# hip-satomi/microbeSEG

Measured on AMD Instinct MI355X. Metric: training crops/sec (256px), higher is better.
Workload: dtype f32; 1 GPU; BASELINE configs[1]: DU-Net distance-map training step, filters [64, 1024], 256x256 crops, per-GPU batch 32, fp32, relu/bn, SmoothL1x2 + Adam(amsgrad); global_batch=32, parallelism=dp1, launch=eager

## Files before the change

include/mseg_hip.h:

```cpp
#ifndef MSEG_HIP_H
#define MSEG_HIP_H

#include <stddef.h>
#include <stdint.h>

#ifdef __cplusplus
extern "C" {
#endif

#define MSEG_OK 0
#define MSEG_EINVAL (-1)
#define MSEG_ELAUNCH (-2)
#define MSEG_EWORKSPACE (-3)

#define MSEG_ACT_NONE 0
#define MSEG_ACT_RELU 1
#define MSEG_ACT_LEAKY 2
#define MSEG_ACT_ELU 3
#define MSEG_ACT_MISH 4

#define MSEG_NORM_BN 0
#define MSEG_NORM_GN 1
#define MSEG_NORM_IN 2

// ... 120 lines not shown
                        const float* running_var, float eps, int C, float* scale, float* shift, void* stream);
int mseg_norm_bwd(const void* gy, const void* z, int N, int HW, int C, int st, int act, int norm, const float* gamma,
                  const float* mean, const float* rstd, void* dz, float* dgamma, float* dbeta, float* dbias,
                  const void* act_in , void* ws, void* stream);

int mseg_maxpool2x2_fwd(const MsegSrc* src, int N, int H, int W, float* out, void* stream);
int mseg_maxpool2x2_bwd(const MsegSrc* src, int N, int H, int W, const float* gout, float* gin, int accumulate,
                        void* stream);

int mseg_head_fwd(const MsegSrc* src, int N, int HW, const float* w, const float* b, int Co, float* out_nchw,
                  void* stream);
size_t mseg_head_bwd_workspace_bytes(int N, int HW, int C, int Co);
int mseg_head_bwd(const MsegSrc* src, int N, int HW, const float* w, int Co, const float* gout_nchw, void* gy,
                  int gy_dtype , float* dW, float* db, void* ws,
                  void* stream);

int mseg_softmax3_hwc(const float* logits_chw, int Hp, int Wp, int pad_y, int pad_x, float* probs_hwc, void* stream);

size_t mseg_loss_workspace_bytes(size_t n);
int mseg_regression_loss(const float* pred, const float* target, size_t n, int kind, float* loss_out,
                         void* ws, void* stream);
int mseg_regression_loss_bwd(const float* pred, const float* target, size_t n, int kind, const float* gscale_dev,
                             float* grad, void* stream);
int mseg_ce_dice_fwd(const float* logits, const int64_t* labels, int N, int HW, int with_dice, double* sums6,
                     double* ce_sum, void* ws, void* stream);
int mseg_ce_dice_bwd(const float* logits, const int64_t* labels, int N, int HW, int with_dice, const double* sums6,
                     double total_px, double dice_weight, const float* gscale_dev, float* grad, void* stream);

int mseg_polygons_find(const uint16_t* labels, int H, int W, int32_t* cand_px, int32_t* cand_id, int32_t* cand_len,
                       int capacity, int32_t* n_cand_dev, void* stream);
// ... 136 lines not shown
```

microbeseg_amd/_lib.py:

```python
import ctypes as C
import os
import pathlib

_HERE = pathlib.Path(__file__).resolve().parent
LIB_PATH = _HERE / "libmseg_hip.so"

ACT = {"none": 0, "relu": 1, "leakyrelu": 2, "elu": 3, "mish": 4}
NORM = {"bn": 0, "gn": 1, "in": 2}
MODE_CONV, MODE_TCONV = 0, 1
EPI_PLAIN, EPI_SCATTER2X2 = 0, 1
MORDER_LINEAR, MORDER_PARITY = 0, 1
ST_F32, ST_BF16 = 0, 1
PIX_U8, PIX_U16, PIX_I32, PIX_F32 = 0, 1, 2, 3
GATHER_RAW, GATHER_F32, GATHER_NORM, GATHER_I64 = 0, 1, 2, 3


class MsegLibraryError(RuntimeError):
    pass


class MsegSrc(C.Structure):
    _fields_ = [("ptr", C.c_void_p), ("scale", C.c_void_p), ("shift", C.c_void_p),
                ("C", C.c_int32), ("act", C.c_int32), ("ss", C.c_int32), ("dtype", C.c_int32)]

# ... 67 lines not shown
    "mseg_pack_job_blocks": (C.c_uint, [_I, _I, _I]),
    "mseg_pack_weights_multi": (_I, [_P, _I, C.c_uint, _P]),
    "mseg_norm_workspace_bytes": (_SZ, [_I, _I, _I]),
    "mseg_norm_set_tails": (_I, [_I]),
    "mseg_norm_set_finish": (_I, [_I]),
    "mseg_norm_stats_from_conv": (_I, [_P, _I, _I, C.c_longlong, _P, _P, _F, _P, _P, _P, _P, _P, _P, _F, _P, _P]),
    "mseg_norm_stats": (_I, [_P, _I, _I, _I, _I, _I, _I, _P, _P, _F, _P, _P, _P, _P, _P, _P, _F, _P, _P, _P]),
    "mseg_activation": (_I, [_P, _I, _I, _I, _I, _I, _P, _P]),
    "mseg_bn_eval_coeffs": (_I, [_P, _P, _P, _P, _F, _I, _P, _P, _P]),
    "mseg_norm_bwd": (_I, [_P, _P, _I, _I, _I, _I, _I, _I, _P, _P, _P, _P, _P, _P, _P, _P, _P, _P]),
    "mseg_maxpool2x2_fwd": (_I, [C.POINTER(MsegSrc), _I, _I, _I, _P, _P]),
    "mseg_maxpool2x2_bwd": (_I, [C.POINTER(MsegSrc), _I, _I, _I, _P, _P, _I, _P]),
    "mseg_head_fwd": (_I, [C.POINTER(MsegSrc), _I, _I, _P, _P, _I, _P, _P]),
    "mseg_head_bwd_workspace_bytes": (_SZ, [_I, _I, _I, _I]),
    "mseg_head_bwd": (_I, [C.POINTER(MsegSrc), _I, _I, _P, _I, _P, _P, _I, _P, _P, _P, _P]),
    "mseg_softmax3_hwc": (_I, [_P, _I, _I, _I, _I, _P, _P]),
    "mseg_loss_workspace_bytes": (_SZ, [_SZ]),
    "mseg_regression_loss": (_I, [_P, _P, _SZ, _I, _P, _P, _P]),
    "mseg_regression_loss_bwd": (_I, [_P, _P, _SZ, _I, _P, _P, _P]),
    "mseg_ce_dice_fwd": (_I, [_P, _P, _I, _I, _I, _P, _P, _P, _P]),
    "mseg_ce_dice_bwd": (_I, [_P, _P, _I, _I, _I, _P, C.c_double, C.c_double, _P, _P, _P]),
    "mseg_adam_amsgrad_step": (_I, [_P, _P, _P, _P, _P, _SZ, _D, _D, _D, _D, _I, _P]),
    "mseg_adam_amsgrad_step_dev": (_I, [_P, _P, _P, _P, _P, _SZ, _P, _D, _D, _D, _P]),
    "mseg_ranger_step": (_I, [_P, _P, _P, _P, _P, _SZ, _I, _D, _D, _D, _D, _I, _I, _I, _D, _P]),
    "mseg_ranger_step_multi": (_I, [_P, _I, _D, _D, _D, _D, _P]),
    "mseg_postproc_workspace_bytes": (_SZ, [_I, _I]),
    "mseg_postproc_tuning": (_I, [_I, _I, _I]),
    "mseg_postproc_set_const_stream": (_I, [_I]),
    "mseg_distance_postprocess": (_I, [_P, _P, _I, _I, _F, _F, _I, _P, _P, _P, _P, _SZ, _P]),
    "mseg_boundary_postprocess": (_I, [_P, _I, _I, _P, _P, _P, _P, _SZ, _P]),
# ... 92 lines not shown
```

microbeseg_amd/csrc/common.h:

```cpp
#pragma once
#include <hip/hip_runtime.h>
#include <stdint.h>
#include "../../include/mseg_hip.h"

extern "C" void mseg_set_hip_error(int e);
extern "C" int mseg_dispatch_dry(void);

#define MSEG_LAUNCH_CHECK()                           \
  do {                                                \
    if (mseg_dispatch_dry()) break;                   \
    hipError_t e__ = hipGetLastError();               \
    if (e__ != hipSuccess) {                          \
      mseg_set_hip_error((int)e__);                   \
      return MSEG_ELAUNCH;                            \
    }                                                 \
  } while (0)

extern "C" void mseg_note_launch(const char* kernel, unsigned grid, unsigned block, int aux);
extern "C" void mseg_dispatch_begin(int dry);
extern "C" void mseg_dispatch_end(MsegKernelInfo* info);
extern "C" void mseg_dispatch_note(int precision, size_t workspace);
extern "C" void mseg_dispatch_note_stats(int rows);
#define MSEG_KL(K, grid_, block_, shmem_, st_, ...)                                              \
  do {                                                                                           \
// ... 152 lines not shown
__device__ __forceinline__ float raw_frame_norm(unsigned v, float fmin, float frange) {
  return __fsub_rn(__fdiv_rn(__fmul_rn(2.f, __fsub_rn((float)v, fmin)), frange), 1.f);
}

__device__ __forceinline__ unsigned xcd_logical_id(unsigned hw_id, unsigned nwg) {
  const unsigned q = nwg >> 3, r = nwg & 7u, xcd = hw_id & 7u;
  return (xcd < r ? xcd * (q + 1u) : r * (q + 1u) + (xcd - r) * q) + (hw_id >> 3);
}

__device__ __forceinline__ float clamp_lo(float v, float lo) {
  float r;
  asm("v_max_f32 %0, %1, %2" : "=v"(r) : "v"(v), "v"(lo));
  return r;
}

__device__ __forceinline__ double wave_sum(double v) {
#pragma unroll
  for (int o = 32; o > 0; o >>= 1) v += __shfl_xor(v, o, 64);
  return v;
}
```

microbeseg_amd/csrc/head.hip:

```cpp
#include "common.h"

#define HEAD_MAXCO 4

template <bool S16, int CO>
__global__ __launch_bounds__(256) void head_fwd_kernel(const MsegSrc s, int N, int HW, const float* __restrict__ w,
                                                       const float* __restrict__ b, int Co, int lpp,
                                                       float* __restrict__ out) {
  constexpr int V = S16 ? 8 : 4, U = 4;
  const int CV = s.C / V;
  const long long total = (long long)N * HW;
  const int sub = threadIdx.x % lpp;
  const long long ppb = blockDim.x / lpp;
  for (long long base = (long long)blockIdx.x * ppb * U; base < total; base += (long long)gridDim.x * ppb * U) {
    float acc[U][CO];
#pragma unroll
    for (int u = 0; u < U; ++u)
#pragma unroll
      for (int co = 0; co < CO; ++co) acc[u][co] = 0.f;
    for (int cv = sub; cv < CV; cv += lpp) {
      uint4 raw[U];
#pragma unroll
      for (int u = 0; u < U; ++u) {
        const long long pix = base + u * ppb + threadIdx.x / lpp;
        const size_t e = (size_t)(pix < total ? pix : 0) * s.C + cv * V;
// ... 157 lines not shown
          float yv[V], o[V];
          if (S16) {
            yv[0] = bf16_lo(yraw[u].x); yv[1] = bf16_hi(yraw[u].x); yv[2] = bf16_lo(yraw[u].y); yv[3] = bf16_hi(yraw[u].y);
            yv[V - 4] = bf16_lo(yraw[u].z); yv[V - 3] = bf16_hi(yraw[u].z); yv[V - 2] = bf16_lo(yraw[u].w); yv[V - 1] = bf16_hi(yraw[u].w);
          } else {
            yv[0] = __uint_as_float(yraw[u].x); yv[1] = __uint_as_float(yraw[u].y);
            yv[2] = __uint_as_float(yraw[u].z); yv[3] = __uint_as_float(yraw[u].w);
          }
#pragma unroll
          for (int j = 0; j < V; j += 4) {
            const float4 a = act_fwd4(make_float4(yv[j], yv[j + 1], yv[j + 2], yv[j + 3]), s.act);
            yv[j] = a.x; yv[j + 1] = a.y; yv[j + 2] = a.z; yv[j + 3] = a.w;
          }
          if (s.scale) {
#pragma unroll
            for (int j = 0; j < V; ++j) yv[j] = yv[j] * sc[j] + sh[j];
          }
#pragma unroll
          for (int j = 0; j < V; ++j) o[j] = 0.f;
#pragma unroll
          for (int co = 0; co < CO; ++co) {
            if (co < g.Co) {
              const float gvc = gv[u][co];
#pragma unroll
              for (int j = 0; j < V; ++j) {
                o[j] += gvc * wv[co][j];
                dw[co][j] += (double)gvc * yv[j];
              }
              if (cv == 0) dbs[co] += gvc;
            }
          }
          if (V == 8 && gy_dtype == MSEG_ST_BF16) {
            *reinterpret_cast<uint4*>(reinterpret_cast<uint16_t*>(gy) + off) =
                make_uint4(pack_bf16x2(o[0], o[1]), pack_bf16x2(o[2], o[3]), pack_bf16x2(o[V - 4], o[V - 3]),
                           pack_bf16x2(o[V - 2], o[V - 1]));
          } else {
#pragma unroll
            for (int j = 0; j < V; j += 4) st_f4_rt(gy, off + j, make_float4(o[j], o[j + 1], o[j + 2], o[j + 3]), gy_dtype);
          }
        }
      }
    }
#pragma unroll
// ... 44 lines not shown
  const int i = blockIdx.x * 8 + o;
  double s = 0.0;
  if (i < total) {
    const int slot = (i < g.Co * g.C) ? i : HEAD_MAXCO * g.C + (i - g.Co * g.C);
    for (int k = kg; k < blocks; k += 32) s += part[(size_t)k * per + slot];
  }
  red[kg][o] = s;
  __syncthreads();
  if (kg == 0 && i < total) {
    double t = 0.0;
#pragma unroll
    for (int j = 0; j < 32; ++j) t += red[j][o];
    if (i < g.Co * g.C) dW[i] = (float)t;
    else if (db) db[i - g.Co * g.C] = (float)t;
  }
}

extern "C" int mseg_head_bwd(const MsegSrc* src, int N, int HW, const float* w, int Co, const float* gout_nchw,
                             void* gy, int gy_dtype, float* dW, float* db, void* ws, void* stream) {
  if (!src || !src->ptr || !w || !gout_nchw || !gy || !dW || !ws) return MSEG_EINVAL;
  if (gy_dtype != MSEG_ST_F32 && gy_dtype != MSEG_ST_BF16) return MSEG_EINVAL;
  if (N <= 0 || HW <= 0 || Co <= 0 || Co > HEAD_MAXCO || src->C <= 0 || (src->C & 3)) return MSEG_EINVAL;
  HeadGeom g = head_geom(N, HW, src->C, Co);
  hipStream_t st = (hipStream_t)stream;
#define HEAD_BWD(CO_, U_, S16_) hipLaunchKernelGGL((head_bwd_kernel<CO_, U_, S16_>), dim3(g.chunks, N), dim3(256), 0, st, *src, g, \
                                                   w, gout_nchw, gy, gy_dtype, (double*)ws)
  if (src->dtype == MSEG_ST_BF16) {
    if (src->C & 7) return MSEG_EINVAL;
    if (Co == 1) HEAD_BWD(1, 2, true); else if (Co == 2) HEAD_BWD(2, 2, true); else HEAD_BWD(4, 1, true);
  } else {
    if (Co == 1) HEAD_BWD(1, 4, false); else if (Co == 2) HEAD_BWD(2, 2, false); else HEAD_BWD(4, 1, false);
  }
#undef HEAD_BWD
  MSEG_LAUNCH_CHECK();
  hipLaunchKernelGGL(head_bwd_reduce_kernel, dim3((Co * (src->C + 1) + 7) / 8), dim3(256), 0, st,
                     (const double*)ws, g, dW, db);
  MSEG_LAUNCH_CHECK();
  return MSEG_OK;
}

__global__ void softmax3_hwc_kernel(const float* __restrict__ logits, int Hp, int Wp, int py, int px, int H, int W,
                                    float* __restrict__ probs) {
  const size_t n = (size_t)H * W;
  const size_t i = (size_t)blockIdx.x * blockDim.x + threadIdx.x;
  if (i >= n) return;
  const int y = (int)(i / W), x = (int)(i - (size_t)y * W);
  const size_t src = (size_t)(y + py) * Wp + (x + px);
  const size_t plane = (size_t)Hp * Wp;
  const float l0 = logits[src], l1 = logits[plane + src], l2 = logits[2 * plane + src];
  const float m = fmaxf(l0, fmaxf(l1, l2));
  const float e0 = expf(l0 - m), e1 = expf(l1 - m), e2 = expf(l2 - m);
// ... 16 lines not shown
```

microbeseg_amd/csrc/norm.hip:

```cpp
#include "common.h"
#include <stdlib.h>

struct NormGeom {
  int N, HW, C, chunks, rows_per_chunk;
  int cw, slices;
};

#define NORM_CTR_BYTES 65536
#define NORM_CTR_MAX (NORM_CTR_BYTES / 4)

static NormGeom norm_geom(int N, int HW, int C, int vec = 4) {
  NormGeom g;
  g.N = N; g.HW = HW; g.C = C;
  const int C4 = C / vec;
  g.cw = C4 < 16 ? (C4 > 0 ? C4 : 1) : 16;
  g.slices = (C4 + g.cw - 1) / g.cw;
  const int rpi = 256 / g.cw;
  const int min_rows = 8 * rpi;
  const int target = 1024;
  int want = (target + N * g.slices - 1) / (N * g.slices > 0 ? N * g.slices : 1);
  int chunks = HW / min_rows;
  if (chunks > want) chunks = want;
  if (chunks < 1) chunks = 1;
  g.rows_per_chunk = (HW + chunks - 1) / chunks;
// ... 365 lines not shown
        }
      } else {
        const double mu = t.mean[c2], r = t.rstd[c2], ga = t.gamma ? (double)t.gamma[c2] : 1.0;
        const double sx = r * (b0 - mu * a0);
        const double m1 = ga * a0 / cnt, m2 = ga * sx / cnt;
        t.k1[c2] = (float)(ga * r);
        t.k2[c2] = (float)(-r * r * m2);
        t.k3[c2] = (float)(-r * m1 + r * r * m2 * mu);
        if (t.dgamma) t.dgamma[c2] = (float)sx;
        if (t.dbeta) t.dbeta[c2] = (float)a0;
      }
    }
  }
}

__device__ __forceinline__ void norm_reduce_chunks_body(const double* __restrict__ part, double* __restrict__ nc,
                                                        const NormGeom& g, int ns, bool handoff, double (*red)[32]) {
  const int o = threadIdx.x & 31, kg = threadIdx.x >> 5;
  const int total = ns * g.N * g.C;
  for (int base = blockIdx.x * 32; base < total; base += gridDim.x * 32) {
    const int i = base + o;
    double acc = 0.0;
    int c = 0, n = 0, sidx = 0;
    if (i < total) {
      c = i % g.C;
      n = (i / g.C) % g.N;
      sidx = i / (g.C * g.N);
      for (int k = kg; k < g.chunks; k += 8) acc += part[(((size_t)n * g.chunks + k) * 3 + sidx) * g.C + c];
    }
    red[kg][o] = acc;
// ... 419 lines not shown
            (const float*)nullptr, 0, g, act, (double*)nullptr, aio_, t);
  MSEG_LAUNCH_CHECK();
  return MSEG_OK;
}

extern "C" int mseg_bn_eval_coeffs(const float* gamma, const float* beta, const float* running_mean,
                                   const float* running_var, float eps, int C, float* scale, float* shift,
                                   void* stream) {
  if (!running_mean || !running_var || !scale || !shift || C <= 0) return MSEG_EINVAL;
  hipLaunchKernelGGL(bn_eval_coeffs_kernel, dim3((C + 255) / 256), dim3(256), 0, (hipStream_t)stream, gamma, beta,
                     running_mean, running_var, eps, C, scale, shift);
  MSEG_LAUNCH_CHECK();
  return MSEG_OK;
}

extern "C" int mseg_norm_bwd(const void* gy, const void* z, int N, int HW, int C, int st_, int act, int norm,
                             const float* gamma, const float* mean, const float* rstd, void* dz, float* dgamma,
                             float* dbeta, float* dbias, const void* act_in, void* ws, void* stream) {
  if (!gy || !z || !mean || !rstd || !dz || !ws || N <= 0 || HW <= 0 || C <= 0 || (C & 3)) return MSEG_EINVAL;
  if ((st_ != MSEG_ST_F32 && st_ != MSEG_ST_BF16) || (st_ == MSEG_ST_BF16 && (C & 7))) return MSEG_EINVAL;
  if (norm < 0 || norm > 2) return MSEG_EINVAL;
  if (norm == MSEG_NORM_GN && (C % 8)) return MSEG_EINVAL;
  hipStream_t st = (hipStream_t)stream;
  NormGeom g = norm_geom(N, HW, C, norm_vec(st_));
  double* part = (double*)((char*)ws + NORM_CTR_BYTES);
  double* nc = part + (size_t)N * g.chunks * 3 * C;
  float* k1 = (float*)(nc + (size_t)3 * N * C);
  float* k2 = k1 + (size_t)N * C;
  float* k3 = k2 + (size_t)N * C;
  const int kss = (norm == MSEG_NORM_BN) ? 0 : C;
  const bool tails = norm_tails_fit(g);
  NormTail t = {};
  t.kind = (tails && norm == MSEG_NORM_BN) ? NORM_TAIL_BN_BWD : NORM_TAIL_NONE;
  t.norm = norm; t.ctr = (unsigned*)ws; t.nc = nc; t.gamma = gamma; t.mean = mean; t.rstd = rstd;
  t.k1 = k1; t.k2 = k2; t.k3 = k3; t.dgamma = dgamma; t.dbeta = dbeta;
  NORM_PASS(1, const_cast<void*>(act_in), z, gy, (void*)nullptr, (const float*)nullptr, (const float*)nullptr,
            (const float*)nullptr, 0, g, act, part, aio_, t);
  MSEG_LAUNCH_CHECK();
  if (t.kind == NORM_TAIL_NONE && norm == MSEG_NORM_BN && norm_finish_fits(C)) {
    NormTail tf = t;
    tf.kind = NORM_TAIL_BN_BWD;
    norm_launch_finish((const double*)part, nc, g, 2, tf, N, C, st);
    MSEG_LAUNCH_CHECK();
  } else if (t.kind == NORM_TAIL_NONE) {
    hipLaunchKernelGGL(norm_reduce_chunks_kernel, dim3(nblocks((size_t)2 * N * C * 8, 4096u)), dim3(256), 0, st,
                       (const double*)part, nc, g, 2);
    MSEG_LAUNCH_CHECK();
    hipLaunchKernelGGL(norm_bwd_finalize_kernel, dim3(nblocks(norm == MSEG_NORM_BN ? C : (size_t)N * C)), dim3(256), 0,
                       st, (const double*)nc, g, norm, gamma, mean, rstd, k1, k2, k3, dgamma, dbeta);
    MSEG_LAUNCH_CHECK();
  }
  double* part2 = part;
  NormTail t2 = {};
  t2.kind = (tails && dbias) ? NORM_TAIL_COLSUM : NORM_TAIL_NONE;
  t2.norm = norm; t2.ctr = (unsigned*)ws; t2.nc = nc; t2.colsum = dbias;
  NORM_PASS(2, const_cast<void*>(act_in), z, gy, dz, (const float*)k1, (const float*)k2, (const float*)k3, kss, g, act,
            part2, aio_, t2);
  MSEG_LAUNCH_CHECK();
  if (dbias && t2.kind == NORM_TAIL_NONE && norm_finish_fits(C)) {
    NormTail tf = t2;
    tf.kind = NORM_TAIL_COLSUM;
    norm_launch_finish((const double*)part2, nc, g, 1, tf, N, C, st);
    MSEG_LAUNCH_CHECK();
  } else if (dbias && t2.kind == NORM_TAIL_NONE) {
    hipLaunchKernelGGL(norm_reduce_chunks_kernel, dim3(nblocks((size_t)N * C * 8, 4096u)), dim3(256), 0, st,
                       (const double*)part2, nc, g, 1);
    MSEG_LAUNCH_CHECK();
    hipLaunchKernelGGL(norm_colsum_kernel, dim3(nblocks(C)), dim3(256), 0, st, (const double*)nc, g, dbias);
    MSEG_LAUNCH_CHECK();
  }
  return MSEG_OK;
}

__global__ void maxpool_fwd_kernel(const MsegSrc s, int N, int H, int W, float* __restrict__ out) {
  const int Ho = H >> 1, Wo = W >> 1, C4 = s.C >> 2;
  const size_t total = (size_t)N * Ho * Wo * C4;
  for (size_t i = (size_t)blockIdx.x * blockDim.x + threadIdx.x; i < total; i += (size_t)gridDim.x * blockDim.x) {
    const int c = (int)(i % C4) * 4;
    size_t r = i / C4;
    const int x = (int)(r % Wo); r /= Wo;
    const int y = (int)(r % Ho);
    const int n = (int)(r / Ho);
    float4 best;
#pragma unroll
    for (int k = 0; k < 4; ++k) {
      const size_t pix = ((size_t)n * H + 2 * y + (k >> 1)) * W + 2 * x + (k & 1);
      float4 v = *reinterpret_cast<const float4*>(s.ptr + pix * s.C + c);
      v = src_transform4(v, s, n, c);
// ... 68 lines not shown
```

microbeseg_amd/engine.py:

```python
import ctypes as C
import os

import torch

from . import _lib
from ._lib import (ACT, NORM, MODE_CONV, MODE_TCONV, EPI_PLAIN, EPI_SCATTER2X2, MORDER_LINEAR, MORDER_PARITY,
                   ST_F32, ST_BF16, MsegSrc, MsegIgemm, MsegWgrad, MsegKernelInfo, check)

BN_EPS = 1e-5
BN_MOMENTUM = 0.1


def _ptr(t):
    return None if t is None else t.data_ptr()


def _stream():
    return torch.cuda.current_stream().cuda_stream


def _pad4(c):
    return (c + 3) // 4 * 4


def _st(t):
    return ST_BF16 if t.dtype == torch.bfloat16 else ST_F32


class Node:
    __slots__ = ("z", "a", "N", "H", "W", "C", "act", "norm", "scale", "shift", "ss", "mean", "rstd", "layer", "inputs",
                 "grad")

    def __init__(self, z, N, H, W, C):
        self.z, self.N, self.H, self.W, self.C = z, N, H, W, C
        self.a = None
        self.act, self.norm = 0, None
        self.scale = self.shift = self.mean = self.rstd = None
        self.ss = 0
        self.layer, self.inputs, self.grad = None, (), None

    def src(self, transform=True):
        s = MsegSrc()
        s.ptr = self.z.data_ptr()
        s.C = self.C
        s.dtype = _st(self.z)
        if transform:
            if self.a is not None:
                s.ptr = self.a.data_ptr()
                s.act = ACT["none"]
            else:
                s.act = self.act
            s.scale = _ptr(self.scale)
            s.shift = _ptr(self.shift)
            s.ss = self.ss
# ... 531 lines not shown
                                  node.rstd.data_ptr(), _ptr(running_mean), _ptr(running_var), BN_MOMENTUM,
                                  _ptr(node.a), w.data_ptr(), _stream()), "norm_stats")
    if running_mean is not None:
        torch.autograd.graph.increment_version((running_mean, running_var))
        note_training_step()


def norm_bwd(node, gy, gamma, dgamma, dbeta, dbias, ws):
    lib = _lib.load()
    N, HW, Cc = node.N, node.H * node.W, node.C
    w = ws.get("norm", lib.mseg_norm_workspace_bytes(N, HW, Cc), zero=True)
    check(lib.mseg_norm_bwd(gy.data_ptr(), node.z.data_ptr(), N, HW, Cc, _st(node.z), node.act, node.norm, _ptr(gamma),
                            node.mean.data_ptr(), node.rstd.data_ptr(), gy.data_ptr(), _ptr(dgamma), _ptr(dbeta),
                            _ptr(dbias), _ptr(node.a), w.data_ptr(), _stream()), "norm_bwd")
    return gy


class ConvSpec:

    def __init__(self, kind, conv, norm_mod, act, norm):
        self.kind = kind
        self.conv = conv
        self.norm_mod = norm_mod
        self.act = ACT[act]
        self.norm = NORM[norm]

    def params(self):
        ps = [self.conv.weight, self.conv.bias]
        if self.norm in (NORM["bn"], NORM["gn"]):
            ps += [self.norm_mod.weight, self.norm_mod.bias]
# ... 269 lines not shown


_wgrad_overlap = os.environ.get("MSEG_WGRAD_OVERLAP", "1") != "0"
_side_streams = {}


def set_wgrad_overlap(flag):
    global _wgrad_overlap
    _wgrad_overlap = bool(flag)


def get_wgrad_overlap():
    return _wgrad_overlap


_overlap_in_capture = os.environ.get("MSEG_OVERLAP_IN_CAPTURE", "0") == "1"


_decoder_overlap = os.environ.get("MSEG_DECODER_OVERLAP", "0") == "1"


def set_decoder_overlap(flag):
    global _decoder_overlap
    _decoder_overlap = bool(flag)


def get_decoder_overlap():
    return _decoder_overlap


# ... 32 lines not shown
    def on_side(dz, fn):
        if side is None:
            return fn(ws)
        ev = torch.cuda.Event()
        ev.record(main)
        with torch.cuda.stream(side):
            side.wait_event(ev)
            fn(_SideWs(ws))
        held.append(dz)
        held_bytes[0] += dz.numel() * dz.element_size()
        if held_bytes[0] > _SIDE_HOLD_BYTES:
            main.wait_stream(side)
            held.clear()
            held_bytes[0] = 0

    for (head, node), go in zip(tape.heads, grad_outs):
        hc = head.conv
        co = hc.weight.shape[0]
        if go is None:
            go = torch.zeros((node.N, co, node.H, node.W), dtype=torch.float32, device=node.z.device)
        go = go.contiguous().float()
        gy = torch.empty_like(node.z)
        dW = _grad_buf(hc.weight, direct)
        db = _grad_buf(hc.bias, direct)
        w = ws.get("head", lib.mseg_head_bwd_workspace_bytes(node.N, node.H * node.W, node.C, co))
        s = node.src()
        check(lib.mseg_head_bwd(C.byref(s), node.N, node.H * node.W, hc.weight.detach().data_ptr(), co,
                                go.data_ptr(), gy.data_ptr(), _st(gy), dW.data_ptr(), db.data_ptr(), w.data_ptr(),
                                _stream()), "head_bwd")
        assert node.grad is None
        node.grad = gy
        grads[id(hc.weight)] = dW
        grads[id(hc.bias)] = db
        if on_grads is not None:
            on_grads([dW, db])

    for node in reversed(tape.nodes):
        sp = node.layer
        gy = node.grad
        node.grad = None
        if gy is None:
            raise RuntimeError("internal: node without gradient")
        if sp is _MaxPoolMarker:
            i0 = node.inputs[0]
            tgt, acc = _accumulate_target(i0, None)
            s = i0.src()
            check(lib.mseg_maxpool2x2_bwd(C.byref(s), i0.N, i0.H, i0.W, gy.data_ptr(), tgt.data_ptr(), acc, _stream()),
                  "maxpool_bwd")
            continue
        conv = sp.conv
        nm = sp.norm_mod
        has_affine = sp.norm in (NORM["bn"], NORM["gn"])
        dgamma = _grad_buf(nm.weight, direct) if has_affine else None
        dbeta = _grad_buf(nm.bias, direct) if has_affine else None
        dbias = _grad_buf(conv.bias, direct)
        dz = norm_bwd(node, gy, nm.weight.detach() if has_affine else None, dgamma, dbeta, dbias, ws)
        if has_affine:
            grads[id(nm.weight)] = dgamma
            grads[id(nm.bias)] = dbeta
        grads[id(conv.bias)] = dbias
        wt = conv.weight.detach()
        dW = _grad_buf(conv.weight, direct)
        ins = node.inputs
        i0 = ins[0]
        N = node.N
        if sp.kind == "up":
            cin, cout = wt.shape[0], wt.shape[1]
            on_side(dz, lambda w_, i0=i0, dz=dz, dW=dW, cout=cout, node=node: wgrad(
                i0.src(), [plain_src(dz, cout)], dW, N, i0.H, i0.W, node.H, node.W, 2, 2, 2, 0, w_))
            wp = pack_weight(conv.weight, 4, cin, cout, 1, cout * 4, 4, kind="dgrad")
            tgt, acc = _accumulate_target(i0, None)
# ... 92 lines not shown
```

Baseline: 244.3 crops/s.

## Fuse head 1x1-conv backward into final norm backward passes

Adds a fused head+norm backward path. The head's input gradient (gout·W) is recomputed on the fly inside the norm statistics and apply kernels instead of being materialized as a full gy tensor. The head weight and bias gradients are accumulated in the same stats pass. This removes one full-resolution write and read of gy and one separate head-backward kernel at the largest 256x256 resolution. The cost is extra per-element FMA work that is done twice, a larger workspace that must be zero-initialized, and eligibility checks in the backward schedule.

New measurement: 245.3 crops/s (median of 6 runs). About the same (+0.4%).

```diff
diff --git a/include/mseg_hip.h b/include/mseg_hip.h
--- a/include/mseg_hip.h
+++ b/include/mseg_hip.h
@@ -158,6 +158,12 @@
 int mseg_head_bwd(const MsegSrc* src, int N, int HW, const float* w, int Co, const float* gout_nchw, void* gy,
                   int gy_dtype , float* dW, float* db, void* ws,
                   void* stream);
+
+size_t mseg_head_norm_bwd_workspace_bytes(int N, int HW, int C, int Co);
+int mseg_head_norm_bwd(const float* gout_nchw, const float* w, int Co, const float* scale, const float* shift, int ss,
+                       const void* z, int N, int HW, int C, int st, int act, int norm, const float* gamma, const float* mean,
+                       const float* rstd, void* dz, float* dgamma, float* dbeta, float* dbias, float* dW_head, float* db_head,
+                       const void* act_in, void* ws, void* stream);
 
 int mseg_softmax3_hwc(const float* logits_chw, int Hp, int Wp, int pad_y, int pad_x, float* probs_hwc, void* stream);
 
diff --git a/microbeseg_amd/_lib.py b/microbeseg_amd/_lib.py
--- a/microbeseg_amd/_lib.py
+++ b/microbeseg_amd/_lib.py
@@ -105,6 +105,9 @@
     "mseg_head_fwd": (_I, [C.POINTER(MsegSrc), _I, _I, _P, _P, _I, _P, _P]),
     "mseg_head_bwd_workspace_bytes": (_SZ, [_I, _I, _I, _I]),
     "mseg_head_bwd": (_I, [C.POINTER(MsegSrc), _I, _I, _P, _I, _P, _P, _I, _P, _P, _P, _P]),
+    "mseg_head_norm_bwd_workspace_bytes": (_SZ, [_I, _I, _I, _I]),
+    "mseg_head_norm_bwd": (_I, [_P, _P, _I, _P, _P, _I, _P, _I, _I, _I, _I, _I, _I, _P, _P, _P, _P, _P, _P, _P, _P, _P, _P, _P,
+                                _P]),
     "mseg_softmax3_hwc": (_I, [_P, _I, _I, _I, _I, _P, _P]),
     "mseg_loss_workspace_bytes": (_SZ, [_SZ]),
     "mseg_regression_loss": (_I, [_P, _P, _SZ, _I, _P, _P, _P]),
diff --git a/microbeseg_amd/csrc/common.h b/microbeseg_amd/csrc/common.h
--- a/microbeseg_amd/csrc/common.h
+++ b/microbeseg_amd/csrc/common.h
@@ -190,6 +190,23 @@
   return r;
 }
 
+#define HEAD_MAXCO 4
+template <int CO, int V>
+__device__ __forceinline__ void head_gy(const float (&gv)[CO], const float (&wv)[CO][V], int Co, float (&o)[V]) {
+#pragma unroll
+  for (int j = 0; j < V; ++j) o[j] = 0.f;
+#pragma unroll
+  for (int co = 0; co < CO; ++co) {
+    if (co < Co) {
+      const float gvc = gv[co];
+#pragma unroll
+      for (int j = 0; j < V; ++j) o[j] = fmaf(gvc, wv[co][j], o[j]);
+    }
+  }
+}
+__attribute__((visibility("hidden"))) void head_bwd_reduce_launch(const double* part, int N, int chunks, int C, int Co,
+                                                                  float* dW, float* db, hipStream_t st);
+
 __device__ __forceinline__ double wave_sum(double v) {
 #pragma unroll
   for (int o = 32; o > 0; o >>= 1) v += __shfl_xor(v, o, 64);
diff --git a/microbeseg_amd/csrc/head.hip b/microbeseg_amd/csrc/head.hip
--- a/microbeseg_amd/csrc/head.hip
+++ b/microbeseg_amd/csrc/head.hip
@@ -1,6 +1,4 @@
 #include "common.h"
-
-#define HEAD_MAXCO 4
 
 template <bool S16, int CO>
 __global__ __launch_bounds__(256) void head_fwd_kernel(const MsegSrc s, int N, int HW, const float* __restrict__ w,
@@ -195,19 +193,15 @@
           }
           if (s.scale) {
 #pragma unroll
-            for (int j = 0; j < V; ++j) yv[j] = yv[j] * sc[j] + sh[j];
-          }
-#pragma unroll
-          for (int j = 0; j < V; ++j) o[j] = 0.f;
+            for (int j = 0; j < V; ++j) yv[j] = fmaf(yv[j], sc[j], sh[j]);
+          }
+          head_gy<CO, V>(gv[u], wv, g.Co, o);
 #pragma unroll
           for (int co = 0; co < CO; ++co) {
             if (co < g.Co) {
               const float gvc = gv[u][co];
 #pragma unroll
-              for (int j = 0; j < V; ++j) {
-                o[j] += gvc * wv[co][j];
-                dw[co][j] += (double)gvc * yv[j];
-              }
+              for (int j = 0; j < V; ++j) dw[co][j] += (double)gvc * yv[j];
               if (cv == 0) dbs[co] += gvc;
             }
           }
@@ -282,6 +276,12 @@
     if (i < g.Co * g.C) dW[i] = (float)t;
     else if (db) db[i - g.Co * g.C] = (float)t;
   }
+}
+
+void head_bwd_reduce_launch(const double* part, int N, int chunks, int C, int Co, float* dW, float* db, hipStream_t st) {
+  HeadGeom g = {};
+  g.N = N; g.C = C; g.Co = Co; g.chunks = chunks;
+  hipLaunchKernelGGL(head_bwd_reduce_kernel, dim3((Co * (C + 1) + 7) / 8), dim3(256), 0, st, part, g, dW, db);
 }
 
 extern "C" int mseg_head_bwd(const MsegSrc* src, int N, int HW, const float* w, int Co, const float* gout_nchw,
@@ -301,8 +301,7 @@
   }
 #undef HEAD_BWD
   MSEG_LAUNCH_CHECK();
-  hipLaunchKernelGGL(head_bwd_reduce_kernel, dim3((Co * (src->C + 1) + 7) / 8), dim3(256), 0, st,
-                     (const double*)ws, g, dW, db);
+  head_bwd_reduce_launch((const double*)ws, N, g.chunks, src->C, Co, dW, db, st);
   MSEG_LAUNCH_CHECK();
   return MSEG_OK;
 }
diff --git a/microbeseg_amd/csrc/norm.hip b/microbeseg_amd/csrc/norm.hip
--- a/microbeseg_amd/csrc/norm.hip
+++ b/microbeseg_amd/csrc/norm.hip
@@ -403,6 +403,270 @@
   }
 }
 
+template <int NS, int V>
+__device__ __forceinline__ void norm_combine_store(double (&s0)[V], double (&s1)[V], double* red, const NormGeom& g,
+                                                   double* pout, int c4, int C4) {
+  const int tid = threadIdx.x;
+  const int CW = g.cw;
+  const int rpi = 256 / CW;
+  const int cq = tid % CW, r0 = tid / CW;
+  double t0[V], t1[V];
+  const bool fold = (CW & (CW - 1)) == 0;
+  if (fold) {
+    for (int m = CW; m < 64; m <<= 1) {
+#pragma unroll
+      for (int j = 0; j < V; ++j) {
+        s0[j] += __shfl_xor(s0[j], m, 64);
+        if (NS == 2) s1[j] += __shfl_xor(s1[j], m, 64);
+      }
+    }
+    const int lane = tid & 63, wv = tid >> 6;
+    if (lane < CW) {
+#pragma unroll
+      for (int j = 0; j < V; ++j) {
+        red[(wv * CW + lane) * 2 * V + j] = s0[j];
+        red[(wv * CW + lane) * 2 * V + V + j] = s1[j];
+      }
+    }
+    __syncthreads();
+    if (tid < CW) {
+#pragma unroll
+      for (int j = 0; j < V; ++j) { t0[j] = red[tid * 2 * V + j]; t1[j] = red[tid * 2 * V + V + j]; }
+#pragma unroll
+      for (int w = 1; w < 4; ++w)
+#pragma unroll
+        for (int j = 0; j < V; ++j) {
+          t0[j] += red[(w * CW + tid) * 2 * V + j];
+          t1[j] += red[(w * CW + tid) * 2 * V + V + j];
+        }
+    }
+  } else {
+#pragma unroll
+    for (int j = 0; j < V; ++j) {
+      red[tid * 2 * V + j] = s0[j];
+      red[tid * 2 * V + V + j] = s1[j];
+    }
+    __syncthreads();
+    if (r0 == 0 && c4 < C4) {
+#pragma unroll
+      for (int j = 0; j < V; ++j) { t0[j] = 0.0; t1[j] = 0.0; }
+      for (int k = 0; k < rpi; ++k) {
+#pragma unroll
+        for (int j = 0; j < V; ++j) {
+          t0[j] += red[(k * CW + cq) * 2 * V + j];
+          t1[j] += red[(k * CW + cq) * 2 * V + V + j];
+        }
+      }
+    }
+  }
+  if (r0 == 0 && c4 < C4) {
+#pragma unroll
+    for (int j = 0; j < V; ++j) {
+      pout[c4 * V + j] = t0[j];
+      if (NS == 2) pout[g.C + c4 * V + j] = t1[j];
+    }
+  }
+}
+
+struct HeadFuse {
+  const float* gout; const float* w;
+  const float* scale; const float* shift;
+  int Co, ss;
+  double* hpart;
+};
+
+template <int CO, bool S16>
+__global__ __launch_bounds__(256) void head_norm_sums_kernel(const void* __restrict__ z, const HeadFuse h, NormGeom g, int act,
+                                                             double* __restrict__ part) {
+  constexpr int V = S16 ? 8 : 4;
+  __shared__ double red[256 * 2 * V];
+  const int tid = threadIdx.x;
+  const int chunk = blockIdx.x, n = blockIdx.y, slice = blockIdx.z;
+  const int C4 = g.C / V;
+  const int CW = g.cw;
+  const int rpi = 256 / CW;
+  const int cq = tid % CW, r0 = tid / CW;
+  const int row_begin = chunk * g.rows_per_chunk;
+  int row_end = row_begin + g.rows_per_chunk;
+  if (row_end > g.HW) row_end = g.HW;
+  double* pout = part + ((size_t)n * g.chunks + chunk) * 3 * g.C;
+  double* hout = h.hpart + ((size_t)n * g.chunks + chunk) * (HEAD_MAXCO * (g.C + 1));
+  const int c4 = slice * CW + cq;
+  const bool active = (c4 < C4) && (r0 < rpi);
+  double s0[V], s1[V], dw[CO][V], dbs[CO];
+#pragma unroll
+  for (int j = 0; j < V; ++j) { s0[j] = 0.0; s1[j] = 0.0; }
+#pragma unroll
+  for (int co = 0; co < CO; ++co) {
+    dbs[co] = 0.0;
+#pragma unroll
+    for (int j = 0; j < V; ++j) dw[co][j] = 0.0;
+  }
+  if (active) {
+    const int c = c4 * V;
+    float wv[CO][V], sc[V], sh[V];
+#pragma unroll
+    for (int co = 0; co < CO; ++co)
+#pragma unroll
+      for (int j = 0; j < V; ++j) wv[co][j] = co < h.Co ? h.w[(size_t)co * g.C + c + j] : 0.f;
+#pragma unroll
+    for (int j = 0; j < V; ++j) {
+      sc[j] = h.scale ? h.scale[(size_t)n * h.ss + c + j] : 1.f;
+      sh[j] = h.scale ? h.shift[(size_t)n * h.ss + c + j] : 0.f;
+    }
+    constexpr int U = 4;
+    for (int r = row_begin + r0; r < row_end; r += rpi * U) {
+      NormVec<S16> zv[U];
+      float gq[U][CO];
+      bool ok[U];
+      float p0[V], p1[V];
+#pragma unroll
+      for (int j = 0; j < V; ++j) { p0[j] = 0.f; p1[j] = 0.f; }
+#pragma unroll
+      for (int u = 0; u < U; ++u) {
+        const int ru = r + u * rpi;
+        ok[u] = ru < row_end;
+        const int rr = ok[u] ? ru : r;
+        zv[u].load(z, ((size_t)n * g.HW + rr) * g.C + c);
+#pragma unroll
+        for (int co = 0; co < CO; ++co) gq[u][co] = co < h.Co ? h.gout[((size_t)n * h.Co + co) * g.HW + rr] : 0.f;
+      }
+#pragma unroll
+      for (int u = 0; u < U; ++u) {
+        if (!ok[u]) continue;
+        float zf[V], a4[V], gf[V];
+        zv[u].get(zf);
+#pragma unroll
+        for (int j = 0; j < V; j += 4) {
+          const float4 t4 = act_fwd4(make_float4(zf[j], zf[j + 1], zf[j + 2], zf[j + 3]), act);
+          a4[j] = t4.x; a4[j + 1] = t4.y; a4[j + 2] = t4.z; a4[j + 3] = t4.w;
+        }
+        head_gy<CO, V>(gq[u], wv, h.Co, gf);
+        NormVec<S16>::round(gf);
+#pragma unroll
+        for (int j = 0; j < V; ++j) { p0[j] += gf[j]; p1[j] = fmaf(gf[j], a4[j], p1[j]); }
+        if (h.scale) {
+#pragma unroll
+          for (int j = 0; j < V; ++j) a4[j] = fmaf(a4[j], sc[j], sh[j]);
+        }
+#pragma unroll
+        for (int co = 0; co < CO; ++co) {
+          if (co < h.Co) {
+            const float gvc = gq[u][co];
+#pragma unroll
+            for (int j = 0; j < V; ++j) dw[co][j] += (double)gvc * a4[j];
+            if (c4 == 0) dbs[co] += gvc;
+          }
+        }
+      }
+#pragma unroll
+      for (int j = 0; j < V; ++j) { s0[j] += (double)p0[j]; s1[j] += (double)p1[j]; }
+    }
+  }
+  norm_combine_store<2, V>(s0, s1, red, g, pout, c4, C4);
+#pragma unroll
+  for (int co = 0; co < CO; ++co) {
+    if (co >= h.Co) break;
+    __syncthreads();
+#pragma unroll
+    for (int j = 0; j < V; ++j) red[tid * V + j] = dw[co][j];
+    if (slice == 0) red[256 * V + tid] = (cq == 0 && r0 < rpi) ? dbs[co] : 0.0;
+    __syncthreads();
+    if (r0 == 0 && c4 < C4) {
+      double t[V];
+#pragma unroll
+      for (int j = 0; j < V; ++j) t[j] = 0.0;
+      for (int k = 0; k < rpi; ++k)
+#pragma unroll
+        for (int j = 0; j < V; ++j) t[j] += red[(k * CW + cq) * V + j];
+#pragma unroll
+      for (int j = 0; j < V; ++j) hout[(size_t)co * g.C + c4 * V + j] = t[j];
+    }
+    if (slice == 0 && tid == 0) {
+      double t = 0.0;
+      for (int k = 0; k < rpi; ++k) t += red[256 * V + k * CW];
+      hout[(size_t)HEAD_MAXCO * g.C + co] = t;
+    }
+  }
+}
+
+template <int CO, bool S16>
+__global__ __launch_bounds__(256) void head_norm_apply_kernel(const void* __restrict__ z, const HeadFuse h,
+                                                              void* __restrict__ dz, const float* __restrict__ k1,
+                                                              const float* __restrict__ k2, const float* __restrict__ k3,
+                                                              int kss, NormGeom g, int act, double* __restrict__ part) {
+  constexpr int V = S16 ? 8 : 4;
+  __shared__ double red[256 * 2 * V];
+  const int tid = threadIdx.x;
+  const int chunk = blockIdx.x, n = blockIdx.y, slice = blockIdx.z;
+  const int C4 = g.C / V;
+  const int CW = g.cw;
+  const int rpi = 256 / CW;
+  const int cq = tid % CW, r0 = tid / CW;
+  const int row_begin = chunk * g.rows_per_chunk;
+  int row_end = row_begin + g.rows_per_chunk;
+  if (row_end > g.HW) row_end = g.HW;
+  double* pout = part + ((size_t)n * g.chunks + chunk) * 3 * g.C;
+  const int c4 = slice * CW + cq;
+  const bool active = (c4 < C4) && (r0 < rpi);
+  double s0[V], s1[V];
+#pragma unroll
+  for (int j = 0; j < V; ++j) { s0[j] = 0.0; s1[j] = 0.0; }
+  if (active) {
+    const int c = c4 * V;
+    float wv[CO][V], a1[V], a2[V], a3[V];
+#pragma unroll
+    for (int co = 0; co < CO; ++co)
+#pragma unroll
+      for (int j = 0; j < V; ++j) wv[co][j] = co < h.Co ? h.w[(size_t)co * g.C + c + j] : 0.f;
+#pragma unroll
+    for (int j = 0; j < V; ++j) {
+      a1[j] = k1[(size_t)n * kss + c + j]; a2[j] = k2[(size_t)n * kss + c + j]; a3[j] = k3[(size_t)n * kss + c + j];
+    }
+    constexpr int U = S16 ? 2 : 4;
+    for (int r = row_begin + r0; r < row_end; r += rpi * U) {
+      NormVec<S16> zv[U];
+      float gq[U][CO];
+      bool ok[U];
+      float p0[V];
+#pragma unroll
+      for (int j = 0; j < V; ++j) p0[j] = 0.f;
+#pragma unroll
+      for (int u = 0; u < U; ++u) {
+        const int ru = r + u * rpi;
+        ok[u] = ru < row_end;
+        const int rr = ok[u] ? ru : r;
+        zv[u].load(z, ((size_t)n * g.HW + rr) * g.C + c);
+#pragma unroll
+        for (int co = 0; co < CO; ++co) gq[u][co] = co < h.Co ? h.gout[((size_t)n * h.Co + co) * g.HW + rr] : 0.f;
+      }
+#pragma unroll
+      for (int u = 0; u < U; ++u) {
+        if (!ok[u]) continue;
+        const size_t off = ((size_t)n * g.HW + r + u * rpi) * g.C + c;
+        float zf[V], a4[V], gf[V], d[V];
+        zv[u].get(zf);
+#pragma unroll
+        for (int j = 0; j < V; j += 4) {
+          const float4 t4 = act_fwd4(make_float4(zf[j], zf[j + 1], zf[j + 2], zf[j + 3]), act);
+          a4[j] = t4.x; a4[j + 1] = t4.y; a4[j + 2] = t4.z; a4[j + 3] = t4.w;
+        }
+        head_gy<CO, V>(gq[u], wv, h.Co, gf);
+        NormVec<S16>::round(gf);
+#pragma unroll
+        for (int j = 0; j < V; ++j)
+          d[j] = (a1[j] * gf[j] + a2[j] * a4[j] + a3[j]) * (S16 ? act_bwd_fast(zf[j], act) : act_bwd(zf[j], act));
+        NormVec<S16>::put(dz, off, d);
+#pragma unroll
+        for (int j = 0; j < V; ++j) p0[j] += d[j];
+      }
+#pragma unroll
+      for (int j = 0; j < V; ++j) s0[j] += (double)p0[j];
+    }
+  }
+  norm_combine_store<1, V>(s0, s1, red, g, pout, c4, C4);
+}
+
 __device__ __forceinline__ void norm_reduce_chunks_body(const double* __restrict__ part, double* __restrict__ nc,
                                                         const NormGeom& g, int ns, bool handoff, double (*red)[32]) {
   const int o = threadIdx.x & 31, kg = threadIdx.x >> 5;
@@ -852,14 +1116,23 @@
   return MSEG_OK;
 }
 
-extern "C" int mseg_norm_bwd(const void* gy, const void* z, int N, int HW, int C, int st_, int act, int norm,
-                             const float* gamma, const float* mean, const float* rstd, void* dz, float* dgamma,
-                             float* dbeta, float* dbias, const void* act_in, void* ws, void* stream) {
-  if (!gy || !z || !mean || !rstd || !dz || !ws || N <= 0 || HW <= 0 || C <= 0 || (C & 3)) return MSEG_EINVAL;
-  if ((st_ != MSEG_ST_F32 && st_ != MSEG_ST_BF16) || (st_ == MSEG_ST_BF16 && (C & 7))) return MSEG_EINVAL;
-  if (norm < 0 || norm > 2) return MSEG_EINVAL;
-  if (norm == MSEG_NORM_GN && (C % 8)) return MSEG_EINVAL;
-  hipStream_t st = (hipStream_t)stream;
+#define HEAD_NORM_PASS(KERNEL_, ...)                                                                                 \
+  do {                                                                                                               \
+    const dim3 grid_(g.chunks, N, g.slices);                                                                         \
+    if (st_ == MSEG_ST_BF16) {                                                                                       \
+      if (hf->Co == 1) hipLaunchKernelGGL((KERNEL_<1, true>), grid_, dim3(256), 0, st, __VA_ARGS__);                 \
+      else if (hf->Co == 2) hipLaunchKernelGGL((KERNEL_<2, true>), grid_, dim3(256), 0, st, __VA_ARGS__);            \
+      else hipLaunchKernelGGL((KERNEL_<4, true>), grid_, dim3(256), 0, st, __VA_ARGS__);                             \
+    } else {                                                                                                         \
+      if (hf->Co == 1) hipLaunchKernelGGL((KERNEL_<1, false>), grid_, dim3(256), 0, st, __VA_ARGS__);                \
+      else if (hf->Co == 2) hipLaunchKernelGGL((KERNEL_<2, false>), grid_, dim3(256), 0, st, __VA_ARGS__);           \
+      else hipLaunchKernelGGL((KERNEL_<4, false>), grid_, dim3(256), 0, st, __VA_ARGS__);                            \
+    }                                                                                                                \
+  } while (0)
+
+static int norm_bwd_launch(const void* gy, const HeadFuse* hf, float* dW_head, float* db_head, const void* z, int N, int HW,
+                           int C, int st_, int act, int norm, const float* gamma, const float* mean, const float* rstd, void* dz,
+                           float* dgamma, float* dbeta, float* dbias, const void* act_in, void* ws, hipStream_t st) {
   NormGeom g = norm_geom(N, HW, C, norm_vec(st_));
   double* part = (double*)((char*)ws + NORM_CTR_BYTES);
   double* nc = part + (size_t)N * g.chunks * 3 * C;
@@ -867,14 +1140,19 @@
   float* k2 = k1 + (size_t)N * C;
   float* k3 = k2 + (size_t)N * C;
   const int kss = (norm == MSEG_NORM_BN) ? 0 : C;
-  const bool tails = norm_tails_fit(g);
+  const bool tails = !hf && norm_tails_fit(g);
   NormTail t = {};
   t.kind = (tails && norm == MSEG_NORM_BN) ? NORM_TAIL_BN_BWD : NORM_TAIL_NONE;
   t.norm = norm; t.ctr = (unsigned*)ws; t.nc = nc; t.gamma = gamma; t.mean = mean; t.rstd = rstd;
   t.k1 = k1; t.k2 = k2; t.k3 = k3; t.dgamma = dgamma; t.dbeta = dbeta;
-  NORM_PASS(1, const_cast<void*>(act_in), z, gy, (void*)nullptr, (const float*)nullptr, (const float*)nullptr,
-            (const float*)nullptr, 0, g, act, part, aio_, t);
+  if (hf) HEAD_NORM_PASS(head_norm_sums_kernel, z, *hf, g, act, part);
+  else NORM_PASS(1, const_cast<void*>(act_in), z, gy, (void*)nullptr, (const float*)nullptr, (const float*)nullptr,
+                 (const float*)nullptr, 0, g, act, part, aio_, t);
   MSEG_LAUNCH_CHECK();
+  if (hf) {
+    head_bwd_reduce_launch((const double*)hf->hpart, N, g.chunks, C, hf->Co, dW_head, db_head, st);
+    MSEG_LAUNCH_CHECK();
+  }
   if (t.kind == NORM_TAIL_NONE && norm == MSEG_NORM_BN && norm_finish_fits(C)) {
     NormTail tf = t;
     tf.kind = NORM_TAIL_BN_BWD;
@@ -892,8 +1170,10 @@
   NormTail t2 = {};
   t2.kind = (tails && dbias) ? NORM_TAIL_COLSUM : NORM_TAIL_NONE;
   t2.norm = norm; t2.ctr = (unsigned*)ws; t2.nc = nc; t2.colsum = dbias;
-  NORM_PASS(2, const_cast<void*>(act_in), z, gy, dz, (const float*)k1, (const float*)k2, (const float*)k3, kss, g, act,
-            part2, aio_, t2);
+  if (hf) HEAD_NORM_PASS(head_norm_apply_kernel, z, *hf, dz, (const float*)k1, (const float*)k2, (const float*)k3, kss, g, act,
+                         part2);
+  else NORM_PASS(2, const_cast<void*>(act_in), z, gy, dz, (const float*)k1, (const float*)k2, (const float*)k3, kss, g, act,
+                 part2, aio_, t2);
   MSEG_LAUNCH_CHECK();
   if (dbias && t2.kind == NORM_TAIL_NONE && norm_finish_fits(C)) {
     NormTail tf = t2;
@@ -910,6 +1190,42 @@
   return MSEG_OK;
 }
 
+extern "C" int mseg_norm_bwd(const void* gy, const void* z, int N, int HW, int C, int st_, int act, int norm,
+                             const float* gamma, const float* mean, const float* rstd, void* dz, float* dgamma,
+                             float* dbeta, float* dbias, const void* act_in, void* ws, void* stream) {
+  if (!gy || !z || !mean || !rstd || !dz || !ws || N <= 0 || HW <= 0 || C <= 0 || (C & 3)) return MSEG_EINVAL;
+  if ((st_ != MSEG_ST_F32 && st_ != MSEG_ST_BF16) || (st_ == MSEG_ST_BF16 && (C & 7))) return MSEG_EINVAL;
+  if (norm < 0 || norm > 2) return MSEG_EINVAL;
+  if (norm == MSEG_NORM_GN && (C % 8)) return MSEG_EINVAL;
+  return norm_bwd_launch(gy, nullptr, nullptr, nullptr, z, N, HW, C, st_, act, norm, gamma, mean, rstd, dz, dgamma, dbeta,
+                         dbias, act_in, ws, (hipStream_t)stream);
+}
+
+extern "C" size_t mseg_head_norm_bwd_workspace_bytes(int N, int HW, int C, int Co) {
+  if (N <= 0 || HW <= 0 || C <= 0 || Co <= 0 || Co > HEAD_MAXCO) return 0;
+  NormGeom g4 = norm_geom(N, HW, C, 4), g8 = norm_geom(N, HW, C, 8);
+  const int chunks = g4.chunks > g8.chunks ? g4.chunks : g8.chunks;
+  return mseg_norm_workspace_bytes(N, HW, C) + (size_t)N * chunks * (HEAD_MAXCO * (C + 1)) * sizeof(double);
+}
+
+extern "C" int mseg_head_norm_bwd(const float* gout_nchw, const float* w, int Co, const float* scale, const float* shift,
+                                  int ss, const void* z, int N, int HW, int C, int st_, int act, int norm,
+                                  const float* gamma, const float* mean, const float* rstd, void* dz, float* dgamma,
+                                  float* dbeta, float* dbias, float* dW_head, float* db_head, const void* act_in, void* ws,
+                                  void* stream) {
+  if (!gout_nchw || !w || !dW_head || Co <= 0 || Co > HEAD_MAXCO || (scale == nullptr) != (shift == nullptr)) return MSEG_EINVAL;
+  if (!z || !mean || !rstd || !dz || !ws || N <= 0 || HW <= 0 || C <= 0 || (C & 3)) return MSEG_EINVAL;
+  if ((st_ != MSEG_ST_F32 && st_ != MSEG_ST_BF16) || (st_ == MSEG_ST_BF16 && (C & 7))) return MSEG_EINVAL;
+  if (norm < 0 || norm > 2) return MSEG_EINVAL;
+  if (norm == MSEG_NORM_GN && (C % 8)) return MSEG_EINVAL;
+  if (act_in || (act != MSEG_ACT_NONE && act != MSEG_ACT_RELU)) return MSEG_EINVAL;
+  HeadFuse hf = {};
+  hf.gout = gout_nchw; hf.w = w; hf.scale = scale; hf.shift = shift; hf.Co = Co; hf.ss = ss;
+  hf.hpart = (double*)((char*)ws + mseg_norm_workspace_bytes(N, HW, C));
+  return norm_bwd_launch(nullptr, &hf, dW_head, db_head, z, N, HW, C, st_, act, norm, gamma, mean, rstd, dz, dgamma, dbeta,
+                         dbias, nullptr, ws, (hipStream_t)stream);
+}
+
 __global__ void maxpool_fwd_kernel(const MsegSrc s, int N, int H, int W, float* __restrict__ out) {
   const int Ho = H >> 1, Wo = W >> 1, C4 = s.C >> 2;
   const size_t total = (size_t)N * Ho * Wo * C4;
diff --git a/microbeseg_amd/engine.py b/microbeseg_amd/engine.py
--- a/microbeseg_amd/engine.py
+++ b/microbeseg_amd/engine.py
@@ -29,7 +29,7 @@
 
 class Node:
     __slots__ = ("z", "a", "N", "H", "W", "C", "act", "norm", "scale", "shift", "ss", "mean", "rstd", "layer", "inputs",
-                 "grad")
+                 "grad", "head")
 
     def __init__(self, z, N, H, W, C):
         self.z, self.N, self.H, self.W, self.C = z, N, H, W, C
@@ -38,6 +38,7 @@
         self.scale = self.shift = self.mean = self.rstd = None
         self.ss = 0
         self.layer, self.inputs, self.grad = None, (), None
+        self.head = None
 
     def src(self, transform=True):
         s = MsegSrc()
@@ -599,6 +600,20 @@
                             node.mean.data_ptr(), node.rstd.data_ptr(), gy.data_ptr(), _ptr(dgamma), _ptr(dbeta),
                             _ptr(dbias), _ptr(node.a), w.data_ptr(), _stream()), "norm_bwd")
     return gy
+
+
+def head_norm_bwd(node, go, hc, dW_head, db_head, gamma, dgamma, dbeta, dbias, ws):
+    lib = _lib.load()
+    N, HW, Cc = node.N, node.H * node.W, node.C
+    co = hc.weight.shape[0]
+    w = ws.get("head_norm", lib.mseg_head_norm_bwd_workspace_bytes(N, HW, Cc, co), zero=True)
+    dz = torch.empty_like(node.z)
+    check(lib.mseg_head_norm_bwd(go.data_ptr(), hc.weight.detach().data_ptr(), co, _ptr(node.scale), _ptr(node.shift),
+                                 node.ss, node.z.data_ptr(), N, HW, Cc, _st(node.z), node.act, node.norm, _ptr(gamma),
+                                 node.mean.data_ptr(), node.rstd.data_ptr(), dz.data_ptr(), _ptr(dgamma), _ptr(dbeta),
+                                 _ptr(dbias), dW_head.data_ptr(), db_head.data_ptr(), None, w.data_ptr(), _stream()),
+          "head_norm_bwd")
+    return dz
 
 
 class ConvSpec:
@@ -898,6 +913,18 @@
     return _wgrad_overlap
 
 
+_head_fusion = os.environ.get("MSEG_HEAD_FUSION", "1") != "0"
+
+
+def set_head_fusion(flag):
+    global _head_fusion
+    _head_fusion = bool(flag)
+
+
+def get_head_fusion():
+    return _head_fusion
+
+
 _overlap_in_capture = os.environ.get("MSEG_OVERLAP_IN_CAPTURE", "0") == "1"
 
 
@@ -960,15 +987,28 @@
             held.clear()
             held_bytes[0] = 0
 
+    shared = set()
+    if _head_fusion:
+        shared = {id(i) for n in tape.nodes for i in n.inputs}
+        seen = set()
+        for _, n in tape.heads:
+            (shared if id(n) in seen else seen).add(id(n))
     for (head, node), go in zip(tape.heads, grad_outs):
         hc = head.conv
         co = hc.weight.shape[0]
         if go is None:
             go = torch.zeros((node.N, co, node.H, node.W), dtype=torch.float32, device=node.z.device)
         go = go.contiguous().float()
-        gy = torch.empty_like(node.z)
         dW = _grad_buf(hc.weight, direct)
         db = _grad_buf(hc.bias, direct)
+        grads[id(hc.weight)] = dW
+        grads[id(hc.bias)] = db
+        if _head_fusion and id(node) not in shared and node.a is None and node.act in (ACT["none"], ACT["relu"]) and \
+                node.norm is not None and node.layer is not None and node.layer is not _MaxPoolMarker:
+            assert node.grad is None and node.head is None
+            node.head = (go, hc, dW, db)
+            continue
+        gy = torch.empty_like(node.z)
         w = ws.get("head", lib.mseg_head_bwd_workspace_bytes(node.N, node.H * node.W, node.C, co))
         s = node.src()
         check(lib.mseg_head_bwd(C.byref(s), node.N, node.H * node.W, hc.weight.detach().data_ptr(), co,
@@ -976,8 +1016,6 @@
                                 _stream()), "head_bwd")
         assert node.grad is None
         node.grad = gy
-        grads[id(hc.weight)] = dW
-        grads[id(hc.bias)] = db
         if on_grads is not None:
             on_grads([dW, db])
 
@@ -985,7 +1023,9 @@
         sp = node.layer
         gy = node.grad
         node.grad = None
-        if gy is None:
+        hd = node.head
+        node.head = None
+        if gy is None and hd is None:
             raise RuntimeError("internal: node without gradient")
         if sp is _MaxPoolMarker:
             i0 = node.inputs[0]
@@ -1000,7 +1040,13 @@
         dgamma = _grad_buf(nm.weight, direct) if has_affine else None
         dbeta = _grad_buf(nm.bias, direct) if has_affine else None
         dbias = _grad_buf(conv.bias, direct)
-        dz = norm_bwd(node, gy, nm.weight.detach() if has_affine else None, dgamma, dbeta, dbias, ws)
+        if hd is not None:
+            dz = head_norm_bwd(node, *hd, nm.weight.detach() if has_affine else None, dgamma, dbeta, dbias, ws)
+            if on_grads is not None:
+                on_grads([hd[2], hd[3]])
+            hd = None
+        else:
+            dz = norm_bwd(node, gy, nm.weight.detach() if has_affine else None, dgamma, dbeta, dbias, ws)
         if has_affine:
             grads[id(nm.weight)] = dgamma
             grads[id(nm.bias)] = dbeta
```
